# Yotsuei/ClearConverse

Hardware: AMD Instinct MI355X
Metric: xRT (audio-sec/wall-sec) end-to-end, 30 s 16 kHz clips (higher is better)
Workload: dtype bf16

## Files before the change

### clearconverse_amd/csrc/sepformer.hip

```cpp
#include <math.h>
#include "../../include/ccx.h"
#include "ccx_common.h"
#include "elementwise.h"
#include <type_traits>
#include "gemm_bf16.h"
#include "model_store.h"
#include "sepformer.h"

namespace {

typedef __attribute__((ext_vector_type(4))) short bf16x4v;

__global__ __launch_bounds__(256) void sep_encoder_kernel(const float* __restrict__ mix, long mix_stride,
                                                          const int* __restrict__ tok_utt, const int* __restrict__ tok_pos,
                                                          const int* __restrict__ utt_L, const float* __restrict__ w,
                                                          float* __restrict__ feats, int n_tok) {
  const int tok = blockIdx.x * 4 + (threadIdx.x >> 6), lane = threadIdx.x & 63;
  if (tok >= n_tok) return;
  const int u = tok_utt[tok], l = tok_pos[tok];
  float2 o = make_float2(0.f, 0.f);
  if (l < utt_L[u]) {
    const float* x = mix + (long)u * mix_stride + 8 * l;
    float xs[16];
#pragma unroll
    for (int k = 0; k < 16; k++) xs[k] = x[k];
    float a = 0.f, b = 0.f;
#pragma unroll
    for (int k = 0; k < 16; k++) {
      a = fmaf(w[(2 * lane) * 16 + k], xs[k], a);
      b = fmaf(w[(2 * lane + 1) * 16 + k], xs[k], b);
    }
    o = make_float2(fmaxf(a, 0.f), fmaxf(b, 0.f));
  }
  ((float2*)(feats + (long)tok * 128))[lane] = o;
}

__global__ void sep_block_input_kernel(const float* __restrict__ x, const float* __restrict__ hc, const int* __restrict__ tok_seq,
                                       const int* __restrict__ tok_pos, const float* __restrict__ pe, float* __restrict__ xin,
                                       float* __restrict__ h, int n_tok) {
  const long i = (long)blockIdx.x * blockDim.x + threadIdx.x;
  if (i >= (long)n_tok * 32) return;
  const int tok = (int)(i >> 5), c4 = (int)(i & 31);
  float4 v = ((const float4*)x)[i];
  if (hc) {
    const float4 a = ((const float4*)(hc + (long)tok_seq[tok] * 128))[c4];
    v.x += a.x; v.y += a.y; v.z += a.z; v.w += a.w;
  }
  ((float4*)xin)[i] = v;
  const float4 p = ((const float4*)(pe + (long)tok_pos[tok] * 128))[c4];
  ((float4*)h)[i] = make_float4(v.x + p.x, v.y + p.y, v.z + p.z, v.w + p.w);
}

__global__ __launch_bounds__(256, 2) void sep_attention_kernel(const bf16_t* __restrict__ qkv, const int* __restrict__ seq_start,
                                                            const int* __restrict__ seq_len, bf16_t* __restrict__ out,
                                                            float scale_log2e) {
  const int lane = threadIdx.x & 63, wave = threadIdx.x >> 6;
  const int seq = blockIdx.x, head = blockIdx.y * 4 + wave;
  const int s0 = seq_start[seq], len = seq_len[seq];
  const int l15 = lane & 15, h4 = lane >> 4;
  const int n_qt = (len + 15) >> 4, n_kt = n_qt;
  const bf16_t* base = qkv + (long)s0 * 384 + head * 16;

  auto load_k = [&](int kt) -> bf16x4v {
    int krow = kt * 16 + l15;
    krow = krow < len ? krow : len - 1;
    return *(const bf16x4v*)(base + 128 + (long)krow * 384 + 4 * h4);
  };
  auto load_v = [&](int kt) -> bf16x4v {
    bf16x4v v;
#pragma unroll
    for (int j = 0; j < 4; j++) {
      int vr = kt * 16 + 4 * h4 + j;
      vr = vr < len ? vr : len - 1;
      v[j] = (short)base[256 + (long)vr * 384 + l15];
    }
    return v;
  };
  const bool resident = n_kt <= 10;
  bf16x4v k_all[10], v_all[10];
  if (resident) {
#pragma unroll
    for (int t = 0; t < 10; t++) {
      const int kt = t < n_kt ? t : n_kt - 1;
      k_all[t] = load_k(kt);
      v_all[t] = load_v(kt);
    }
  }

  for (int qt = 0; qt < n_qt; qt++) {
    int qrow = qt * 16 + l15;
    qrow = qrow < len ? qrow : len - 1;
    const bf16x4v qf = *(const bf16x4v*)(base + (long)qrow * 384 + 4 * h4);
    float m_run = -1e30f, l_run = 0.f;
    f32x4 o = {0.f, 0.f, 0.f, 0.f};
    auto key_block = [&](int kt0, int nk, auto full_tag) {
      constexpr bool FULL = decltype(full_tag)::value;
      f32x4 s[10];
      bf16x4v vf[10];
#pragma unroll
      for (int t = 0; t < 10; t++) {
        if (FULL || t < nk) {
          const bf16x4v kf = resident ? k_all[t] : load_k(kt0 + t);
          s[t] = __builtin_amdgcn_mfma_f32_16x16x16bf16_1k(kf, qf, (f32x4){0.f, 0.f, 0.f, 0.f}, 0, 0, 0);
          vf[t] = resident ? v_all[t] : load_v(kt0 + t);
        }
      }
      float mx = -1e30f;
#pragma unroll
      for (int t = 0; t < 10; t++)
        if (FULL || t < nk) {
          if ((kt0 + t) * 16 + 16 > len) {
#pragma unroll
            for (int r = 0; r < 4; r++)
              if ((kt0 + t) * 16 + 4 * h4 + r >= len) s[t][r] = -INFINITY;
          }
#pragma unroll
          for (int r = 0; r < 4; r++) mx = fmaxf(mx, s[t][r]);
        }
      mx = fmaxf(mx, lane_xor16(mx));
      mx = fmaxf(mx, lane_xor32(mx));
      mx = fmaxf(m_run, mx * scale_log2e);
      const float alpha = __builtin_amdgcn_exp2f(m_run - mx);
      m_run = mx;
      float ps = 0.f;
#pragma unroll
      for (int t = 0; t < 10; t++)
        if (FULL || t < nk) {
#pragma unroll
          for (int r = 0; r < 4; r++) {
            const float pv = __builtin_amdgcn_exp2f(fmaf(s[t][r], scale_log2e, -mx));
            s[t][r] = pv;
            ps += pv;
          }
        }
      l_run = l_run * alpha + ps;
      float arow[4];
#pragma unroll
      for (int r = 0; r < 4; r++) arow[r] = __shfl(alpha, 4 * h4 + r, 64);
#pragma unroll
      for (int r = 0; r < 4; r++) o[r] *= arow[r];
#pragma unroll
      for (int t = 0; t < 10; t++)
        if (FULL || t < nk) {
          union { bf16x4v v; uint32_t u[2]; } pa;
          pa.u[0] = pack_bf16x2(s[t][0], s[t][1]);
          pa.u[1] = pack_bf16x2(s[t][2], s[t][3]);
          o = __builtin_amdgcn_mfma_f32_16x16x16bf16_1k(pa.v, vf[t], o, 0, 0, 0);
        }
    };
    for (int kt0 = 0; kt0 < n_kt; kt0 += 10) {
      const int nk = (n_kt - kt0) < 10 ? (n_kt - kt0) : 10;
      if (nk == 10) key_block(kt0, 10, std::true_type{});
      else key_block(kt0, nk, std::false_type{});
    }
    float lt = l_run + lane_xor16(l_run);
    lt += lane_xor32(lt);
#pragma unroll
    for (int r = 0; r < 4; r++) {
      const int q = qt * 16 + 4 * h4 + r;
      const float inv = 1.0f / __shfl(lt, 4 * h4 + r, 64);
      if (q < len) out[(long)(s0 + q) * 128 + head * 16 + l15] = f32_to_bf16(o[r] * inv);
    }
  }
}

__device__ __forceinline__ float2 ln_row128(const float* __restrict__ row, const float* __restrict__ g,
                                            const float* __restrict__ b, int lane) {
  const float2 v = ((const float2*)row)[lane];
  const float mean = wave_reduce_sum(v.x + v.y) * (1.0f / 128.0f);
  const float dx = v.x - mean, dy = v.y - mean;
  const float rstd = rsqrtf(wave_reduce_sum(dx * dx + dy * dy) * (1.0f / 128.0f) + 1e-6f);
  const float2 gg = ((const float2*)g)[lane], bb = ((const float2*)b)[lane];
  return make_float2(dx * rstd * gg.x + bb.x, dy * rstd * gg.y + bb.y);
}

__global__ __launch_bounds__(256) void sep_final_norm_kernel(const float* __restrict__ h, const float* __restrict__ xin,
                                                             const int* __restrict__ seq_start, const int* __restrict__ seq_len,
                                                             const float* __restrict__ ln_g, const float* __restrict__ ln_b,
                                                             const float* __restrict__ gln_g, const float* __restrict__ gln_b,
                                                             float* __restrict__ y) {
  __shared__ float red[8];
  const int seq = blockIdx.x, lane = threadIdx.x & 63, wave = threadIdx.x >> 6;
  const int s0 = seq_start[seq], len = seq_len[seq];
  float sum = 0.f;
  for (int r = wave; r < len; r += 4) {
    const float2 v = ln_row128(h + (long)(s0 + r) * 128, ln_g, ln_b, lane);
    sum += v.x + v.y;
  }
  sum = wave_reduce_sum(sum);
  if (lane == 0) red[wave] = sum;
  __syncthreads();
  const float n = (float)len * 128.0f;
  const float mean = (red[0] + red[1] + red[2] + red[3]) / n;
  float sq = 0.f;
  for (int r = wave; r < len; r += 4) {
    const float2 v = ln_row128(h + (long)(s0 + r) * 128, ln_g, ln_b, lane);
    sq += (v.x - mean) * (v.x - mean) + (v.y - mean) * (v.y - mean);
  }
  sq = wave_reduce_sum(sq);
  if (lane == 0) red[4 + wave] = sq;
  __syncthreads();
  const float rstd = 1.0f / sqrtf((red[4] + red[5] + red[6] + red[7]) / n + 1e-8f);
  const float2 gg = ((const float2*)gln_g)[lane], bb = ((const float2*)gln_b)[lane];
  for (int r = wave; r < len; r += 4) {
    const float2 v = ln_row128(h + (long)(s0 + r) * 128, ln_g, ln_b, lane);
    const float2 xi = ((const float2*)(xin + (long)(s0 + r) * 128))[lane];
    ((float2*)(y + (long)(s0 + r) * 128))[lane] =
        make_float2(gg.x * (v.x - mean) * rstd + bb.x + xi.x, gg.y * (v.y - mean) * rstd + bb.y + xi.y);
  }
}

#define FF_TOK 256
#define FF_HB 64
#define FF_P1 (FF_HB * 256)
#define FF_P2 (128 * FF_HB * 2)
#define FF_STAGE (FF_P1 + FF_P2)
#define FF_NSTAGE 4
#define FF_LDS (FF_NSTAGE * FF_STAGE + 4096)
typedef const __attribute__((address_space(1))) void* ff_gptr_t;
typedef __attribute__((address_space(3))) void* ff_lptr_t;

__device__ __forceinline__ int ff_key1(int r) { return (r & 3) | (((r >> 4) & 3) << 2); }
__device__ __forceinline__ int ff_key2(int r) { return ((r >> 1) & 1) | (((r >> 5) & 1) << 2); }

constexpr int AB_MAX_TOK = CCX_SEP_FUSED_MAX_TOK;
__device__ __forceinline__ int ab_off(int row, int chunk) { return row * 256 + ((chunk ^ (row & 15)) << 4); }

__global__ __launch_bounds__(512) void sep_attn_block_kernel(float* __restrict__ h, const float* __restrict__ ln_g, const float* __restrict__ ln_b,
                                                             const bf16_t* __restrict__ Wqkv, const float* __restrict__ bqkv,
                                                             const bf16_t* __restrict__ Wo, const float* __restrict__ bo,
                                                             const int* __restrict__ seq_start, const int* __restrict__ seq_len,
                                                             float scale_log2e, float eps) {
  __shared__ __attribute__((aligned(16))) char xs[AB_MAX_TOK * 256];
  const int tid = threadIdx.x, lane = tid & 63;
  const int wave = __builtin_amdgcn_readfirstlane(tid >> 6);
  const int l15 = lane & 15, h4 = lane >> 4;
  const int seq = blockIdx.x;
  const int s0 = seq_start[seq], len = seq_len[seq];
  if (len <= 0) return;
  const int n_t = (len + 15) >> 4;

  {
    const float2 g = ((const float2*)ln_g)[lane], b = ((const float2*)ln_b)[lane];
#pragma unroll
    for (int half = 0; half < 2; half++) {
      float2 v[10];
#pragma unroll
      for (int i = 0; i < 10; i++) {
        const int r = wave + 8 * (10 * half + i);
        v[i] = r < len ? ((const float2*)(h + (long)(s0 + r) * 128))[lane] : make_float2(0.f, 0.f);
      }
#pragma unroll
      for (int i = 0; i < 10; i++) {
        const int r = wave + 8 * (10 * half + i);
        const float mean = wave_reduce_sum(v[i].x + v[i].y) * (1.f / 128.f);
        const float dx = v[i].x - mean, dy = v[i].y - mean;
        const float rstd = rsqrtf(wave_reduce_sum(dx * dx + dy * dy) * (1.f / 128.f) + eps);
        uint32_t o = pack_bf16x2(dx * rstd * g.x + b.x, dy * rstd * g.y + b.y);
        if (r >= len) o = 0;
        *(uint32_t*)(xs + ab_off(r, lane >> 2) + (lane & 3) * 4) = o;
      }
    }
  }
  __syncthreads();

  bf16x4v q_all[10], k_all[10], v_all[10];
  {
    bf16x8 wq[4], wk[4];
#pragma unroll
    for (int ks = 0; ks < 4; ks++) {
      const long o = (long)(16 * wave + l15) * 128 + 32 * ks + 8 * h4;
      wq[ks] = *(const bf16x8*)(Wqkv + o);
      wk[ks] = *(const bf16x8*)(Wqkv + 128 * 128 + o);
    }
    const float4 bq = *(const float4*)(bqkv + 16 * wave + 4 * h4);
    const float4 bk = *(const float4*)(bqkv + 128 + 16 * wave + 4 * h4);
#pragma unroll
    for (int t = 0; t < 10; t++) {
      const int tt = t < n_t ? t : n_t - 1;
      f32x4 aq = {0.f, 0.f, 0.f, 0.f}, ak = aq;
#pragma unroll
      for (int ks = 0; ks < 4; ks++) {
        const bf16x8 xf = *(const bf16x8*)(xs + ab_off(16 * tt + l15, 4 * ks + h4));
        aq = __builtin_amdgcn_mfma_f32_16x16x32_bf16(wq[ks], xf, aq, 0, 0, 0);
        ak = __builtin_amdgcn_mfma_f32_16x16x32_bf16(wk[ks], xf, ak, 0, 0, 0);
      }
      union { bf16x4v v; uint32_t u[2]; } c;
      c.u[0] = pack_bf16x2(aq[0] + bq.x, aq[1] + bq.y); c.u[1] = pack_bf16x2(aq[2] + bq.z, aq[3] + bq.w);
      q_all[t] = c.v;
      c.u[0] = pack_bf16x2(ak[0] + bk.x, ak[1] + bk.y); c.u[1] = pack_bf16x2(ak[2] + bk.z, ak[3] + bk.w);
      k_all[t] = c.v;
    }
  }
  {
    bf16x8 wv[4];
#pragma unroll
    for (int ks = 0; ks < 4; ks++) wv[ks] = *(const bf16x8*)(Wqkv + 256 * 128 + (long)(16 * wave + l15) * 128 + 32 * ks + 8 * h4);
    const float bv = bqkv[256 + 16 * wave + l15];
#pragma unroll
    for (int t = 0; t < 10; t++) {
      const int tt = t < n_t ? t : n_t - 1;
      f32x4 av = {0.f, 0.f, 0.f, 0.f};
#pragma unroll
      for (int ks = 0; ks < 4; ks++) {
        const bf16x8 xf = *(const bf16x8*)(xs + ab_off(16 * tt + l15, 4 * ks + h4));
        av = __builtin_amdgcn_mfma_f32_16x16x32_bf16(xf, wv[ks], av, 0, 0, 0);
      }
      union { bf16x4v v; uint32_t u[2]; } c;
      c.u[0] = pack_bf16x2(av[0] + bv, av[1] + bv); c.u[1] = pack_bf16x2(av[2] + bv, av[3] + bv);
      v_all[t] = c.v;
    }
  }
  __syncthreads();

  for (int qt = 0; qt < n_t; qt++) {
    bf16x4v qf = q_all[0];
#pragma unroll
    for (int t = 1; t < 10; t++) qf = (t == qt) ? q_all[t] : qf;
    f32x4 sc[10];
#pragma unroll
    for (int t = 0; t < 10; t++) sc[t] = __builtin_amdgcn_mfma_f32_16x16x16bf16_1k(k_all[t], qf, (f32x4){0.f, 0.f, 0.f, 0.f}, 0, 0, 0);
    float mx = -1e30f;
#pragma unroll
    for (int t = 0; t < 10; t++) {
      if (t * 16 + 16 > len) {
#pragma unroll
        for (int r = 0; r < 4; r++)
          if (t * 16 + 4 * h4 + r >= len) sc[t][r] = -INFINITY;
      }
#pragma unroll
      for (int r = 0; r < 4; r++) mx = fmaxf(mx, sc[t][r]);
    }
    mx = fmaxf(mx, lane_xor16(mx));
    mx = fmaxf(mx, lane_xor32(mx));
    mx *= scale_log2e;
    float ps = 0.f;
    f32x4 o = {0.f, 0.f, 0.f, 0.f};
#pragma unroll
    for (int t = 0; t < 10; t++) {
#pragma unroll
      for (int r = 0; r < 4; r++) {
        const float pv = __builtin_amdgcn_exp2f(fmaf(sc[t][r], scale_log2e, -mx));
        sc[t][r] = pv;
        ps += pv;
      }
      union { bf16x4v v; uint32_t u[2]; } pa;
      pa.u[0] = pack_bf16x2(sc[t][0], sc[t][1]);
      pa.u[1] = pack_bf16x2(sc[t][2], sc[t][3]);
      o = __builtin_amdgcn_mfma_f32_16x16x16bf16_1k(pa.v, v_all[t], o, 0, 0, 0);
    }
    float lt = ps + lane_xor16(ps);
    lt += lane_xor32(lt);
#pragma unroll
    for (int r = 0; r < 4; r++) {
      const int row = qt * 16 + 4 * h4 + r;
      const float inv = 1.0f / __shfl(lt, 4 * h4 + r, 64);
      *(bf16_t*)(xs + ab_off(row, 2 * wave + (l15 >> 3)) + (l15 & 7) * 2) = f32_to_bf16(o[r] * inv);
    }
  }
  __syncthreads();

  {
    bf16x8 wo[4];
#pragma unroll
    for (int ks = 0; ks < 4; ks++) wo[ks] = *(const bf16x8*)(Wo + (long)(16 * wave + l15) * 128 + 32 * ks + 8 * h4);
    const float4 b4 = *(const float4*)(bo + 16 * wave + 4 * h4);
    for (int t = 0; t < n_t; t++) {
      const int tok = 16 * t + l15;
      float4* hp = (float4*)(h + (long)(s0 + (tok < len ? tok : len - 1)) * 128 + 16 * wave + 4 * h4);
      const float4 res = *hp;
      f32x4 acc = {0.f, 0.f, 0.f, 0.f};
#pragma unroll
      for (int ks = 0; ks < 4; ks++) {
        const bf16x8 af = *(const bf16x8*)(xs + ab_off(tok, 4 * ks + h4));
        acc = __builtin_amdgcn_mfma_f32_16x16x32_bf16(wo[ks], af, acc, 0, 0, 0);
      }
      if (tok < len) *hp = make_float4(res.x + acc[0] + b4.x, res.y + acc[1] + b4.y, res.z + acc[2] + b4.z, res.w + acc[3] + b4.w);
    }
  }
}

__global__ __launch_bounds__(512) void sep_ffn_kernel(float* __restrict__ h, const float* __restrict__ ln_g, const float* __restrict__ ln_b,
                                                      const bf16_t* __restrict__ W1, const float* __restrict__ b1,
                                                      const bf16_t* __restrict__ W2, const float* __restrict__ b2, int n_tok, int d_ffn,
                                                      float eps) {
  extern __shared__ __attribute__((aligned(16))) char ff_smem[];
  const int tid = threadIdx.x, lane = tid & 63, wave = tid >> 6;
  const int l15 = lane & 15, hq = lane >> 4;
  const int tok0 = blockIdx.x * FF_TOK + wave * 32;
  const int n_stage = d_ffn / FF_HB;
  float* b1s = (float*)(ff_smem + FF_NSTAGE * FF_STAGE);

  const bf16_t* src1[2];
  const bf16_t* src2[2];
#pragma unroll
  for (int i = 0; i < 2; i++) {
    const int r1 = (wave * 2 + i) * 4 + (lane >> 4);
    src1[i] = W1 + (long)r1 * 128 + (((lane & 15) ^ ff_key1(r1)) << 3);
    const int r2 = (wave * 2 + i) * 8 + (lane >> 3);
    src2[i] = W2 + (long)r2 * d_ffn + (((lane & 7) ^ ff_key2(r2)) << 3);
  }
  auto stage = [&](int st) {
    char* s1 = ff_smem + (st & (FF_NSTAGE - 1)) * FF_STAGE;
    char* s2 = s1 + FF_P1;
#pragma unroll
    for (int i = 0; i < 2; i++)
      __builtin_amdgcn_global_load_lds((ff_gptr_t)(src1[i] + (long)st * FF_HB * 128), (ff_lptr_t)(s1 + (wave * 2 + i) * 1024), 16, 0, 0);
#pragma unroll
    for (int i = 0; i < 2; i++)
      __builtin_amdgcn_global_load_lds((ff_gptr_t)(src2[i] + (long)st * FF_HB), (ff_lptr_t)(s2 + (wave * 2 + i) * 1024), 16, 0, 0);
  };

  bf16x8 xb[2][4];
  {
    float g[32], bt[32];
#pragma unroll
    for (int ob = 0; ob < 2; ob++)
#pragma unroll
      for (int i4 = 0; i4 < 4; i4++) {
        const float4 gv = ((const float4*)(ln_g + 64 * ob + 16 * hq))[i4], bv = ((const float4*)(ln_b + 64 * ob + 16 * hq))[i4];
        g[16 * ob + 4 * i4] = gv.x; g[16 * ob + 4 * i4 + 1] = gv.y; g[16 * ob + 4 * i4 + 2] = gv.z; g[16 * ob + 4 * i4 + 3] = gv.w;
        bt[16 * ob + 4 * i4] = bv.x; bt[16 * ob + 4 * i4 + 1] = bv.y; bt[16 * ob + 4 * i4 + 2] = bv.z; bt[16 * ob + 4 * i4 + 3] = bv.w;
      }
#pragma unroll
    for (int mt = 0; mt < 2; mt++) {
      int tok = tok0 + mt * 16 + l15;
      tok = tok < n_tok ? tok : n_tok - 1;
      const float* xr = h + (long)tok * 128 + 16 * hq;
      float v[32];
#pragma unroll
      for (int ob = 0; ob < 2; ob++)
#pragma unroll
        for (int i4 = 0; i4 < 4; i4++) {
          const float4 t = ((const float4*)(xr + 64 * ob))[i4];
          v[16 * ob + 4 * i4] = t.x; v[16 * ob + 4 * i4 + 1] = t.y; v[16 * ob + 4 * i4 + 2] = t.z; v[16 * ob + 4 * i4 + 3] = t.w;
        }
      float sm = 0.f;
#pragma unroll
      for (int c = 0; c < 32; c++) sm += v[c];
      sm += lane_xor16(sm); sm += lane_xor32(sm);
      const float mean = sm * (1.f / 128.f);
      float sq = 0.f;
#pragma unroll
      for (int c = 0; c < 32; c++) { const float d = v[c] - mean; sq = fmaf(d, d, sq); }
      sq += lane_xor16(sq); sq += lane_xor32(sq);
      const float rstd = rsqrtf(sq * (1.f / 128.f) + eps);
#pragma unroll
      for (int ks = 0; ks < 4; ks++) {
        union { bf16x8 vv; uint32_t u[4]; } cv;
#pragma unroll
        for (int e = 0; e < 4; e++) {
          const int c = 8 * ks + 2 * e;
          cv.u[e] = pack_bf16x2((v[c] - mean) * rstd * g[c] + bt[c], (v[c + 1] - mean) * rstd * g[c + 1] + bt[c + 1]);
        }
        xb[mt][ks] = cv.vv;
      }
    }
  }
  for (int i = tid; i < d_ffn; i += 512) b1s[i] = b1[i];

  f32x4 acc2[2][8];
#pragma unroll
  for (int mt = 0; mt < 2; mt++)
#pragma unroll
    for (int jo = 0; jo < 8; jo++) acc2[mt][jo] = (f32x4){0.f, 0.f, 0.f, 0.f};

  const int rq = 16 * (l15 >> 2) + (l15 & 3);
  const int k1 = l15;
  const int k2 = ((l15 >> 1) & 1) | (((l15 >> 3) & 1) << 2);
  asm volatile("s_waitcnt vmcnt(0)" ::: "memory");
  stage(0);
  if (n_stage > 1) stage(1);
  if (n_stage > 2) stage(2);
  for (int st = 0; st < n_stage; st++) {
    const int ahead = n_stage - 1 - st;
    if (ahead >= 2) asm volatile("s_waitcnt vmcnt(8)" ::: "memory");
    else if (ahead == 1) asm volatile("s_waitcnt vmcnt(4)" ::: "memory");
    else asm volatile("s_waitcnt vmcnt(0)" ::: "memory");
    asm volatile("s_waitcnt lgkmcnt(0)" ::: "memory");
    __builtin_amdgcn_s_barrier();
    if (st + 3 < n_stage) stage(st + 3);
    const char* s1 = ff_smem + (st & (FF_NSTAGE - 1)) * FF_STAGE;
    const char* s2 = s1 + FF_P1;
    f32x4 acc1[2][4];
    f32x4 bv[4];
    {
      const uint32_t baddr = (uint32_t)(uintptr_t)(ff_lptr_t)(b1s + st * FF_HB + 16 * hq);
#pragma unroll
      for (int j = 0; j < 4; j++) asm volatile("ds_read_b128 %0, %1" : "=v"(bv[j]) : "v"(baddr + 16 * j) : "memory");
    }
#pragma unroll
    for (int mt = 0; mt < 2; mt++)
#pragma unroll
      for (int j = 0; j < 4; j++) acc1[mt][j] = (f32x4){0.f, 0.f, 0.f, 0.f};
#pragma unroll
    for (int ks = 0; ks < 4; ks++) {
      const int chunk = 8 * (ks >> 1) + 2 * hq + (ks & 1);
#pragma unroll
      for (int j = 0; j < 4; j++) {
        const bf16x8 w = *(const bf16x8*)(s1 + (rq + 4 * j) * 256 + ((chunk ^ k1) << 4));
        acc1[0][j] = __builtin_amdgcn_mfma_f32_16x16x32_bf16(w, xb[0][ks], acc1[0][j], 0, 0, 0);
        acc1[1][j] = __builtin_amdgcn_mfma_f32_16x16x32_bf16(w, xb[1][ks], acc1[1][j], 0, 0, 0);
      }
    }
    asm volatile("s_waitcnt lgkmcnt(0)" ::: "memory");
    __builtin_amdgcn_sched_barrier(0);
    bf16x8 sf[2][2];
#pragma unroll
    for (int mt = 0; mt < 2; mt++)
#pragma unroll
      for (int sx = 0; sx < 2; sx++) {
        union { bf16x8 vv; uint32_t u[4]; } cv;
        const f32x4 a = acc1[mt][2 * sx] + bv[2 * sx], b = acc1[mt][2 * sx + 1] + bv[2 * sx + 1];
        cv.u[0] = pack_bf16x2(fmaxf(a[0], 0.f), fmaxf(a[1], 0.f)); cv.u[1] = pack_bf16x2(fmaxf(a[2], 0.f), fmaxf(a[3], 0.f));
        cv.u[2] = pack_bf16x2(fmaxf(b[0], 0.f), fmaxf(b[1], 0.f)); cv.u[3] = pack_bf16x2(fmaxf(b[2], 0.f), fmaxf(b[3], 0.f));
        sf[mt][sx] = cv.vv;
      }
#pragma unroll
    for (int sx = 0; sx < 2; sx++) {
      const int chunk = 2 * hq + sx;
#pragma unroll
      for (int jo = 0; jo < 8; jo++) {
        const bf16x8 w = *(const bf16x8*)(s2 + (64 * (jo >> 2) + rq + 4 * (jo & 3)) * 128 + ((chunk ^ k2) << 4));
        acc2[0][jo] = __builtin_amdgcn_mfma_f32_16x16x32_bf16(w, sf[0][sx], acc2[0][jo], 0, 0, 0);
        acc2[1][jo] = __builtin_amdgcn_mfma_f32_16x16x32_bf16(w, sf[1][sx], acc2[1][jo], 0, 0, 0);
      }
    }
  }

#pragma unroll
  for (int mt = 0; mt < 2; mt++) {
    const int tok = tok0 + mt * 16 + l15;
    if (tok >= n_tok) continue;
#pragma unroll
    for (int ob = 0; ob < 2; ob++) {
      float4* hp = (float4*)(h + (long)tok * 128 + 64 * ob + 16 * hq);
      const float4* bp = (const float4*)(b2 + 64 * ob + 16 * hq);
#pragma unroll
      for (int jp = 0; jp < 4; jp++) {
        const float4 r = hp[jp], bv = bp[jp];
        const f32x4 a = acc2[mt][4 * ob + jp];
        hp[jp] = make_float4(a[0] + bv.x + r.x, a[1] + bv.y + r.y, a[2] + bv.z + r.z, a[3] + bv.w + r.w);
      }
    }
  }
}

__global__ __launch_bounds__(128) void sep_chunk_mean_kernel(const float* __restrict__ x, float* __restrict__ mem, int seg) {
  const int chunk = blockIdx.x, c = threadIdx.x;
  const float* p = x + (long)chunk * seg * 128 + c;
  float s = 0.f;
  for (int t = 0; t < seg; t++) s += p[(long)t * 128];
  mem[(long)chunk * 128 + c] = s / (float)seg;
}

__global__ void sep_prelu_bf16_kernel(const float* __restrict__ x, const float* __restrict__ slope, bf16_t* __restrict__ out, long n4) {
  const long i = (long)blockIdx.x * blockDim.x + threadIdx.x;
  if (i >= n4) return;
  const float a = slope[0];
  const float4 v = ((const float4*)x)[i];
  uint2 o;
  o.x = pack_bf16x2(v.x >= 0 ? v.x : a * v.x, v.y >= 0 ? v.y : a * v.y);
  o.y = pack_bf16x2(v.z >= 0 ? v.z : a * v.z, v.w >= 0 ? v.w : a * v.w);
  ((uint2*)out)[i] = o;
}

__global__ __launch_bounds__(256) void sep_decoder_kernel(const float* __restrict__ feats, const float* __restrict__ fc,
                                                          const int* __restrict__ utt_tok0, const int* __restrict__ utt_L,
                                                          const int* __restrict__ utt_T, const float* __restrict__ wdec,
                                                          float* __restrict__ out, long out_stride, int n_utt) {
  const int u = blockIdx.y;
  const int l = blockIdx.x * 4 + (threadIdx.x >> 6), lane = threadIdx.x & 63;
  const int T = utt_T[u], L = utt_L[u];
  const long t0 = 8L * l;
  if (t0 >= out_stride) return;
  float2* dst = (float2*)(out + ((long)u * out_stride + t0) * 2);
  if (t0 >= T || l > L) {
    if (lane < 8 && t0 + lane < out_stride) dst[lane] = make_float2(0.f, 0.f);
    return;
  }
  float g[2][2][2];
#pragma unroll
  for (int dl = 0; dl < 2; dl++) {
    const int ll = l - dl;
    const bool ok = ll >= 0 && ll < L;
    const long tok = utt_tok0[u] + (ok ? ll : 0);
    const float2 f = ((const float2*)(feats + tok * 128))[lane];
    const float4 m = ((const float4*)(fc + tok * 256))[lane];
    const float z = ok ? 1.f : 0.f;
    g[dl][0][0] = z * f.x * fmaxf(m.x, 0.f); g[dl][0][1] = z * f.y * fmaxf(m.z, 0.f);
    g[dl][1][0] = z * f.x * fmaxf(m.y, 0.f); g[dl][1][1] = z * f.y * fmaxf(m.w, 0.f);
  }
  float4 w0[4], w1[4];
#pragma unroll
  for (int i = 0; i < 4; i++) {
    w0[i] = ((const float4*)(wdec + (2 * lane) * 16))[i];
    w1[i] = ((const float4*)(wdec + (2 * lane + 1) * 16))[i];
  }
  const float* w0f = (const float*)w0;
  const float* w1f = (const float*)w1;
  float2 res = make_float2(0.f, 0.f);
#pragma unroll
  for (int k = 0; k < 8; k++) {
    float a0 = g[0][0][0] * w0f[k] + g[0][0][1] * w1f[k];
    float a1 = g[0][1][0] * w0f[k] + g[0][1][1] * w1f[k];
    a0 += g[1][0][0] * w0f[k + 8] + g[1][0][1] * w1f[k + 8];
    a1 += g[1][1][0] * w0f[k + 8] + g[1][1][1] * w1f[k + 8];
    a0 = wave_reduce_sum(a0);
    a1 = wave_reduce_sum(a1);
    if (lane == k) res = make_float2(a0, a1);
  }
  if (lane < 8 && t0 + lane < out_stride) dst[lane] = (t0 + lane < T) ? res : make_float2(0.f, 0.f);
}

struct SepLayer {
  float *ln1_g, *ln1_b, *ln2_g, *ln2_b, *bqkv, *bo, *b1, *b2;
  bf16_t *Wqkv, *Wo, *W1, *W2;
};
struct SepBlock {
  std::vector<SepLayer> layers;
  float *lnf_g, *lnf_b, *gln_g, *gln_b;
};

}

static constexpr float kSepScaleLog2e = 0.25f * 1.4426950408889634f;
static constexpr float kSepLnEps = 1e-6f;

int ccx_launch_sep_attn_block(ccx_ctx* ctx, float* h, const float* ln_g, const float* ln_b, const bf16_t* Wqkv, const float* bqkv,
                              const bf16_t* Wo, const float* bo, const int* seq_start, const int* seq_len, int n_seq, int n_tok,
                              int max_len, hipStream_t st) {
  const int D = 128;
  {
    ccx_prof_scope ps(ctx, st, "sep_attn_block_kernel", 2.0 * n_tok * (double)D * 4 * D + 4.0 * n_tok * (double)max_len * D,
                      2.0 * n_tok * D * 4.0 + 2.0 * 4 * D * D);
    hipLaunchKernelGGL(sep_attn_block_kernel, dim3(n_seq), dim3(512), 0, st, h, ln_g, ln_b, Wqkv, bqkv, Wo, bo, seq_start, seq_len,
                       kSepScaleLog2e, kSepLnEps);
  }
  CCX_CHECK_LAUNCH(ctx);
  return CCX_OK;
}

int ccx_launch_sep_attention(ccx_ctx* ctx, const bf16_t* qkv, const int* seq_start, const int* seq_len, int n_seq, int n_head,
                             bf16_t* out, hipStream_t st) {
  {
    ccx_prof_scope ps(ctx, st, "sep_attention_kernel", 0.0, 0.0);
    hipLaunchKernelGGL(sep_attention_kernel, dim3(n_seq, n_head / 4), dim3(256), 0, st, qkv, seq_start, seq_len, out, kSepScaleLog2e);
  }
  CCX_CHECK_LAUNCH(ctx);
  return CCX_OK;
}

int ccx_launch_sep_ffn(ccx_ctx* ctx, float* h, const float* ln_g, const float* ln_b, const bf16_t* W1, const float* b1,
                       const bf16_t* W2, const float* b2, int n_tok, int d_ffn, hipStream_t st) {
  const int D = 128;
  {
    static ccx_lds_optin optin;
    CCX_HIP(ctx, optin.ensure(ctx->device, (const void*)sep_ffn_kernel, FF_LDS));
    ccx_prof_scope ps(ctx, st, "sep_ffn_kernel", 4.0 * n_tok * (double)D * d_ffn, 2.0 * n_tok * D * 4.0 + 4.0 * D * d_ffn);
    hipLaunchKernelGGL(sep_ffn_kernel, dim3(ccx_cdiv(n_tok, FF_TOK)), dim3(512), FF_LDS, st, h, ln_g, ln_b, W1, b1, W2, b2, n_tok, d_ffn,
                       kSepLnEps);
  }
  CCX_CHECK_LAUNCH(ctx);
  return CCX_OK;
}

int ccx_launch_sep_final_norm(ccx_ctx* ctx, const float* h, const float* xin, const int* seq_start, const int* seq_len, int n_seq,
                              const float* ln_g, const float* ln_b, const float* gln_g, const float* gln_b, float* y, hipStream_t st) {
  hipLaunchKernelGGL(sep_final_norm_kernel, dim3(n_seq), dim3(256), 0, st, h, xin, seq_start, seq_len, ln_g, ln_b, gln_g, gln_b, y);
  CCX_CHECK_LAUNCH(ctx);
  return CCX_OK;
}

int ccx_launch_sep_decoder(ccx_ctx* ctx, const float* feats, const float* fc, const int* utt_tok0, const int* utt_L, const int* utt_T,
                           const float* wdec, float* out, long out_stride, int n_utt, hipStream_t st) {
  hipLaunchKernelGGL(sep_decoder_kernel, dim3(ccx_cdiv(ccx_cdiv((int)out_stride, 8), 4), n_utt), dim3(256), 0, st, feats, fc, utt_tok0, utt_L,
                     utt_T, wdec, out, out_stride, n_utt);
  CCX_CHECK_LAUNCH(ctx);
  return CCX_OK;
}

struct ccx_sepformer {
  ccx_ctx* ctx = nullptr;
  ccx_sepformer_dims d{};
  int max_tokens = 0, max_utts = 0;
  bool finalized = false;
  ccx_dev_store store{"sepformer"};
  float *w_enc = nullptr, *w_dec = nullptr, *prelu = nullptr, *b_fc = nullptr, *pe = nullptr;
  bf16_t* W_fc = nullptr;
  std::vector<SepBlock> seg, mem;
  float *feats = nullptr, *x = nullptr, *xin = nullptr, *h = nullptr, *fc = nullptr, *memx = nullptr, *memxin = nullptr,
        *memh = nullptr, *hc = nullptr;
  bf16_t *xn = nullptr, *qkv = nullptr, *att = nullptr;
  int *tok_utt = nullptr, *tok_pos = nullptr, *tok_chunk = nullptr, *tok_cpos = nullptr, *chunk_start = nullptr,
      *chunk_len = nullptr, *utt_L = nullptr, *utt_T = nullptr, *utt_tok0 = nullptr, *utt_chunk0 = nullptr, *utt_nchunk = nullptr,
      *mem_utt = nullptr, *mem_pos = nullptr;
  int pe_len = 0;
};

namespace {

int load_block(ccx_sepformer* s, const std::string& prefix, SepBlock& B) {
  const int D = s->d.d_model, F = s->d.d_ffn;
  B.layers.resize(s->d.n_layers);
  for (int l = 0; l < s->d.n_layers; l++) {
    const std::string p = prefix + ".mdl.layers." + std::to_string(l);
    SepLayer& L = B.layers[l];
    CCX_NEED(s->store, wi, p + ".self_att.att.in_proj_weight", 3 * D, D); CCX_NEED(s->store, bi, p + ".self_att.att.in_proj_bias", 3 * D);
    CCX_NEED(s->store, wo, p + ".self_att.att.out_proj.weight", D, D); CCX_NEED(s->store, bo, p + ".self_att.att.out_proj.bias", D);
    CCX_NEED(s->store, w1, p + ".pos_ffn.ffn.0.weight", F, D); CCX_NEED(s->store, b1, p + ".pos_ffn.ffn.0.bias", F);
    CCX_NEED(s->store, w2, p + ".pos_ffn.ffn.3.weight", D, F); CCX_NEED(s->store, b2, p + ".pos_ffn.ffn.3.bias", D);
    CCX_NEED(s->store, g1, p + ".norm1.norm.weight", D); CCX_NEED(s->store, be1, p + ".norm1.norm.bias", D);
    CCX_NEED(s->store, g2, p + ".norm2.norm.weight", D); CCX_NEED(s->store, be2, p + ".norm2.norm.bias", D);
    CCX_TRY(s->store.upload_bf16(&L.Wqkv, wi->data)); CCX_TRY(s->store.upload(&L.bqkv, bi->data.data(), 3 * D));
    CCX_TRY(s->store.upload_bf16(&L.Wo, wo->data)); CCX_TRY(s->store.upload(&L.bo, bo->data.data(), D));
    CCX_TRY(s->store.upload_bf16(&L.W1, w1->data)); CCX_TRY(s->store.upload(&L.b1, b1->data.data(), F));
    CCX_TRY(s->store.upload_bf16(&L.W2, w2->data)); CCX_TRY(s->store.upload(&L.b2, b2->data.data(), D));
    CCX_TRY(s->store.upload(&L.ln1_g, g1->data.data(), D)); CCX_TRY(s->store.upload(&L.ln1_b, be1->data.data(), D));
    CCX_TRY(s->store.upload(&L.ln2_g, g2->data.data(), D)); CCX_TRY(s->store.upload(&L.ln2_b, be2->data.data(), D));
  }
  CCX_NEED(s->store, fg, prefix + ".mdl.norm.norm.weight", D); CCX_NEED(s->store, fb, prefix + ".mdl.norm.norm.bias", D);
  CCX_NEED(s->store, gg, prefix + ".norm.weight", D); CCX_NEED(s->store, gb, prefix + ".norm.bias", D);
  CCX_TRY(s->store.upload(&B.lnf_g, fg->data.data(), D)); CCX_TRY(s->store.upload(&B.lnf_b, fb->data.data(), D));
  CCX_TRY(s->store.upload(&B.gln_g, gg->data.data(), D)); CCX_TRY(s->store.upload(&B.gln_b, gb->data.data(), D));
  return CCX_OK;
}

int run_block(ccx_sepformer* s, const SepBlock& B, const float* x, const float* hc, const int* tok_seq, const int* tok_pos,
              const int* seq_start, const int* seq_len, int n_tok, int n_seq, int max_len, float* xin, float* h, float* y, hipStream_t st) {
  ccx_ctx* ctx = s->ctx;
  const int D = s->d.d_model, F = s->d.d_ffn;
  hipLaunchKernelGGL(sep_block_input_kernel, dim3(ccx_cdiv(n_tok * 32, 256)), dim3(256), 0, st, x, hc, tok_seq, tok_pos, s->pe,
                     xin, h, n_tok);
  CCX_CHECK_LAUNCH(ctx);
  const char* fenv = getenv("CCX_SEP_FUSED_ATTN");
  const bool fused = (fenv ? atoi(fenv) != 0 : true) && max_len <= AB_MAX_TOK;
  for (const SepLayer& L : B.layers) {
    GemmParams p;
    if (fused) {
      CCX_TRY(ccx_launch_sep_attn_block(ctx, h, L.ln1_g, L.ln1_b, L.Wqkv, L.bqkv, L.Wo, L.bo, seq_start, seq_len, n_seq, n_tok, max_len, st));
    } else {
    CCX_TRY(ccx_launch_layernorm(ctx, h, D, L.ln1_g, L.ln1_b, s->xn, nullptr, D, n_tok, D, 1e-6f, st));
    memset(&p, 0, sizeof(p));
    p.A = s->xn; p.lda = D; p.W = L.Wqkv; p.ldw = D; p.M = n_tok; p.N = 3 * D; p.K = D; p.bias = L.bqkv; p.out = s->qkv; p.ldo = 3 * D;
    CCX_TRY(ccx_launch_gemm(ctx, EPI_BF16, p, st));
    CCX_TRY(ccx_launch_sep_attention(ctx, s->qkv, seq_start, seq_len, n_seq, s->d.n_head, s->att, st));
    memset(&p, 0, sizeof(p));
    p.A = s->att; p.lda = D; p.W = L.Wo; p.ldw = D; p.M = n_tok; p.N = D; p.K = D; p.bias = L.bo; p.out = h; p.ldo = D; p.resid = h; p.ldr = D;
    CCX_TRY(ccx_launch_gemm(ctx, EPI_F32_RESID, p, st));
    }
    CCX_TRY(ccx_launch_sep_ffn(ctx, h, L.ln2_g, L.ln2_b, L.W1, L.b1, L.W2, L.b2, n_tok, F, st));
  }
  CCX_TRY(ccx_launch_sep_final_norm(ctx, h, xin, seq_start, seq_len, n_seq, B.lnf_g, B.lnf_b, B.gln_g, B.gln_b, y, st));
  return CCX_OK;
}

}

extern "C" {

int ccx_sepformer_create(ccx_ctx* ctx, const ccx_sepformer_dims* dims, int max_tokens, int max_utts, ccx_sepformer** out) {
  if (!ctx) return CCX_ERR_ARG;
  CCX_REQUIRE(ctx, dims && out, "ccx_sepformer_create: null argument");
  const ccx_sepformer_dims& d = *dims;
  CCX_REQUIRE(ctx, d.n_filters == 128 && d.d_model == 128 && d.kernel == 16 && d.stride == 8 && d.n_head == 8 && d.n_spk == 2,
              "sepformer: only the resepformer-wsj02mix geometry (128 filters, k16 s8, d_model 128, 8 heads, 2 speakers) is built");
  CCX_REQUIRE(ctx, d.d_ffn % 128 == 0 && d.d_ffn <= 1024 && d.segment >= 16 && d.n_layers >= 1 && d.n_blocks >= 1, "sepformer: bad dims");
  CCX_REQUIRE(ctx, max_tokens >= d.segment && max_utts >= 1, "sepformer: capacity too small");
  ccx_sepformer* s = new ccx_sepformer();
  s->ctx = ctx; s->store.ctx = ctx; s->d = d;
  s->max_tokens = ccx_cdiv(max_tokens, d.segment) * d.segment;
  s->max_utts = max_utts;
  *out = s;
  return CCX_OK;
}

void ccx_sepformer_destroy(ccx_sepformer* s) {
  if (!s) return;
  s->store.free_all();
  delete s;
}

int ccx_sepformer_set_tensor(ccx_sepformer* s, const char* name, const float* data, int64_t numel) {
  if (!s) return CCX_ERR_ARG;
  CCX_REQUIRE(s->ctx, !s->finalized && name && data && numel > 0, "sepformer: set_tensor bad arguments");
  const std::string nm(name);
  CCX_REQUIRE(s->ctx, nm.rfind("encoder.", 0) == 0 || nm.rfind("decoder.", 0) == 0 || nm.rfind("masknet.", 0) == 0,
              "sepformer: unknown tensor name '%s'", name);
  return s->store.stage(name, data, numel);
}

int ccx_sepformer_finalize(ccx_sepformer* s) {
  if (!s) return CCX_ERR_ARG;
  CCX_REQUIRE(s->ctx, !s->finalized, "sepformer: finalize called twice");
  const ccx_sepformer_dims& d = s->d;
  const int D = d.d_model, F = d.d_ffn, N = d.n_filters;
  {
    CCX_NEED(s->store, we, "encoder.conv1d.weight", N, 1, d.kernel);
    CCX_NEED(s->store, wd, "decoder.weight", N, 1, d.kernel);
    CCX_NEED(s->store, pr, "masknet.model.output_fc.0.weight", 1);
    CCX_NEED(s->store, wf, "masknet.model.output_fc.1.weight", N * d.n_spk, D, 1);
    CCX_NEED(s->store, bf, "masknet.model.output_fc.1.bias", N * d.n_spk);
    CCX_TRY(s->store.upload(&s->w_enc, we->data));
    CCX_TRY(s->store.upload(&s->w_dec, wd->data));
    CCX_TRY(s->store.upload(&s->prelu, pr->data.data(), 1));
    CCX_TRY(s->store.upload_bf16(&s->W_fc, wf->data));
    CCX_TRY(s->store.upload(&s->b_fc, bf->data));
  }
  s->seg.resize(d.n_blocks);
  s->mem.resize(d.n_blocks > 0 ? d.n_blocks - 1 : 0);
  for (int i = 0; i < d.n_blocks; i++) {
    CCX_TRY(load_block(s, "masknet.model.seg_model." + std::to_string(i), s->seg[i]));
    if (i < d.n_blocks - 1) CCX_TRY(load_block(s, "masknet.model.mem_model." + std::to_string(i), s->mem[i]));
  }
  s->store.staged.clear();
  const int max_chunks = s->max_tokens / d.segment;
  s->pe_len = d.segment > max_chunks ? d.segment : max_chunks;
  {
    std::vector<float> pe((size_t)s->pe_len * D);
    for (int p = 0; p < s->pe_len; p++)
      for (int i = 0; i < D; i += 2) {
        const float den = expf((float)i * -(logf(10000.0f) / (float)D));
        pe[(size_t)p * D + i] = sinf((float)p * den);
        pe[(size_t)p * D + i + 1] = cosf((float)p * den);
      }
    CCX_TRY(s->store.upload(&s->pe, pe));
  }
  const size_t T = (size_t)s->max_tokens;
  CCX_TRY(s->store.alloc(&s->feats, T * D, true)); CCX_TRY(s->store.alloc(&s->x, T * D, true)); CCX_TRY(s->store.alloc(&s->xin, T * D, true)); CCX_TRY(s->store.alloc(&s->h, T * D, true));
  CCX_TRY(s->store.alloc(&s->fc, T * 2 * D, true)); CCX_TRY(s->store.alloc(&s->xn, T * D, true)); CCX_TRY(s->store.alloc(&s->qkv, T * 3 * D, true));
  CCX_TRY(s->store.alloc(&s->att, T * D, true));
  CCX_TRY(s->store.alloc(&s->memx, (size_t)max_chunks * D, true)); CCX_TRY(s->store.alloc(&s->memxin, (size_t)max_chunks * D, true));
  CCX_TRY(s->store.alloc(&s->memh, (size_t)max_chunks * D, true)); CCX_TRY(s->store.alloc(&s->hc, (size_t)max_chunks * D, true));
  CCX_TRY(s->store.alloc(&s->tok_utt, T, true)); CCX_TRY(s->store.alloc(&s->tok_pos, T, true)); CCX_TRY(s->store.alloc(&s->tok_chunk, T, true)); CCX_TRY(s->store.alloc(&s->tok_cpos, T, true));
  CCX_TRY(s->store.alloc(&s->chunk_start, (size_t)max_chunks, true)); CCX_TRY(s->store.alloc(&s->chunk_len, (size_t)max_chunks, true));
  CCX_TRY(s->store.alloc(&s->mem_utt, (size_t)max_chunks, true)); CCX_TRY(s->store.alloc(&s->mem_pos, (size_t)max_chunks, true));
  const size_t U = (size_t)s->max_utts;
  CCX_TRY(s->store.alloc(&s->utt_L, U, true)); CCX_TRY(s->store.alloc(&s->utt_T, U, true)); CCX_TRY(s->store.alloc(&s->utt_tok0, U, true)); CCX_TRY(s->store.alloc(&s->utt_chunk0, U, true));
  CCX_TRY(s->store.alloc(&s->utt_nchunk, U, true));
  s->finalized = true;
  return CCX_OK;
}

int ccx_sepformer_separate(ccx_sepformer* s, const float* mix, int64_t stride, const int* n_samples, int B, float* out,
                           void* stream_) {
  if (!s) return CCX_ERR_ARG;
  ccx_ctx* ctx = s->ctx;
  hipStream_t st = (hipStream_t)stream_;
  CCX_REQUIRE(ctx, s->finalized && mix && n_samples && out && B >= 1 && B <= s->max_utts, "sepformer_separate: bad arguments (B=%d, max %d)", B, s->max_utts);
  const ccx_sepformer_dims& d = s->d;
  const int D = d.d_model, seg = d.segment;
  std::vector<int> uL(B), uT(B), utok0(B), uchunk0(B), unchunk(B);
  int n_tok = 0, n_chunk = 0, max_nchunk = 0;
  for (int b = 0; b < B; b++) {
    CCX_REQUIRE(ctx, n_samples[b] >= d.kernel && n_samples[b] <= stride, "sepformer_separate: utterance %d has %d samples (need >= %d, <= stride)", b, n_samples[b], d.kernel);
    uT[b] = n_samples[b];
    uL[b] = (n_samples[b] - d.kernel) / d.stride + 1;
    const int rest = seg - uL[b] % seg;
    unchunk[b] = (uL[b] + rest) / seg;
    utok0[b] = n_tok; uchunk0[b] = n_chunk;
    n_tok += unchunk[b] * seg; n_chunk += unchunk[b];
    max_nchunk = unchunk[b] > max_nchunk ? unchunk[b] : max_nchunk;
  }
  CCX_REQUIRE(ctx, n_tok <= s->max_tokens, "sepformer_separate: %d tokens exceed capacity %d", n_tok, s->max_tokens);
  CCX_REQUIRE(ctx, n_chunk <= s->pe_len, "sepformer_separate: memory sequence too long");
  std::vector<int> t_utt(n_tok), t_pos(n_tok), t_chunk(n_tok), t_cpos(n_tok), c_start(n_chunk), c_len(n_chunk), m_utt(n_chunk), m_pos(n_chunk);
  for (int b = 0; b < B; b++) {
    for (int c = 0; c < unchunk[b]; c++) {
      const int cg = uchunk0[b] + c;
      c_start[cg] = utok0[b] + c * seg; c_len[cg] = seg; m_utt[cg] = b; m_pos[cg] = c;
      for (int i = 0; i < seg; i++) {
        const int t = c_start[cg] + i;
        t_utt[t] = b; t_pos[t] = c * seg + i; t_chunk[t] = cg; t_cpos[t] = i;
      }
    }
  }
#define UP(dst, vec) CCX_HIP(ctx, hipMemcpyAsync(dst, vec.data(), vec.size() * 4, hipMemcpyHostToDevice, st))
  UP(s->tok_utt, t_utt); UP(s->tok_pos, t_pos); UP(s->tok_chunk, t_chunk); UP(s->tok_cpos, t_cpos);
  UP(s->chunk_start, c_start); UP(s->chunk_len, c_len); UP(s->mem_utt, m_utt); UP(s->mem_pos, m_pos);
  UP(s->utt_L, uL); UP(s->utt_T, uT); UP(s->utt_tok0, utok0); UP(s->utt_chunk0, uchunk0); UP(s->utt_nchunk, unchunk);
#undef UP
  CCX_HIP(ctx, hipStreamSynchronize(st));

  hipLaunchKernelGGL(sep_encoder_kernel, dim3(ccx_cdiv(n_tok, 4)), dim3(256), 0, st, mix, (long)stride, s->tok_utt, s->tok_pos,
                     s->utt_L, s->w_enc, s->feats, n_tok);
  CCX_CHECK_LAUNCH(ctx);
  const float* cur = s->feats;
  const float* hc = nullptr;
  for (int i = 0; i < d.n_blocks; i++) {
    CCX_TRY(run_block(s, s->seg[i], cur, hc, s->tok_chunk, s->tok_cpos, s->chunk_start, s->chunk_len, n_tok, n_chunk, seg, s->xin, s->h,
                   s->x, st));
    cur = s->x;
    if (i < d.n_blocks - 1) {
      hipLaunchKernelGGL(sep_chunk_mean_kernel, dim3(n_chunk), dim3(128), 0, st, s->x, s->memx, seg);
      CCX_CHECK_LAUNCH(ctx);
      CCX_TRY(run_block(s, s->mem[i], s->memx, nullptr, s->mem_utt, s->mem_pos, s->utt_chunk0, s->utt_nchunk, n_chunk, B, max_nchunk, s->memxin,
                     s->memh, s->hc, st));
      hc = s->hc;
    }
  }
  hipLaunchKernelGGL(sep_prelu_bf16_kernel, dim3(ccx_cdiv(n_tok * 32, 256)), dim3(256), 0, st, s->x, s->prelu, s->xn, (long)n_tok * 32);
  CCX_CHECK_LAUNCH(ctx);
  GemmParams p;
  memset(&p, 0, sizeof(p));
  p.A = s->xn; p.lda = D; p.W = s->W_fc; p.ldw = D; p.M = n_tok; p.N = 2 * D; p.K = D; p.bias = s->b_fc; p.out = s->fc; p.ldo = 2 * D;
  CCX_TRY(ccx_launch_gemm(ctx, EPI_F32, p, st));
  return ccx_launch_sep_decoder(ctx, s->feats, s->fc, s->utt_tok0, s->utt_L, s->utt_T, s->w_dec, out, (long)stride, B, st);
}

}
```

Measured before the change: 1698.

## Restructure attention block kernel to prefetch weights and residuals early

Loads the K/V weights and biases before LayerNorm and fuses the K and V projections into one loop over tiles. Q weights load partway through that loop, and Q tiles go to shared memory instead of being selected from registers. The Wo weights and residual rows are prefetched before the barrier, and the output projection is fully unrolled with stores deferred. The aim is to hide global-load latency and cut register-select overhead, with a launch bound of 4 and asm pins to steer register allocation. The cost is higher register pressure and full 10-tile unrolling even for short sequences.

```diff
diff --git a/clearconverse_amd/csrc/sepformer.hip b/clearconverse_amd/csrc/sepformer.hip
--- a/clearconverse_amd/csrc/sepformer.hip
+++ b/clearconverse_amd/csrc/sepformer.hip
@@ -226,7 +226,9 @@
 constexpr int AB_MAX_TOK = CCX_SEP_FUSED_MAX_TOK;
 __device__ __forceinline__ int ab_off(int row, int chunk) { return row * 256 + ((chunk ^ (row & 15)) << 4); }
 
-__global__ __launch_bounds__(512) void sep_attn_block_kernel(float* __restrict__ h, const float* __restrict__ ln_g, const float* __restrict__ ln_b,
+#define AB_PIN(a, b) asm volatile("" : "+v"(a), "+v"(b))
+
+__global__ __launch_bounds__(512, 4) void sep_attn_block_kernel(float* __restrict__ h, const float* __restrict__ ln_g, const float* __restrict__ ln_b,
                                                              const bf16_t* __restrict__ Wqkv, const float* __restrict__ bqkv,
                                                              const bf16_t* __restrict__ Wo, const float* __restrict__ bo,
                                                              const int* __restrict__ seq_start, const int* __restrict__ seq_len,
@@ -240,6 +242,16 @@
   if (len <= 0) return;
   const int n_t = (len + 15) >> 4;
 
+  bf16x8 wk[4], wv[4];
+#pragma unroll
+  for (int ks = 0; ks < 4; ks++) {
+    const long o = (long)(16 * wave + l15) * 128 + 32 * ks + 8 * h4;
+    wk[ks] = *(const bf16x8*)(Wqkv + 128 * 128 + o);
+    wv[ks] = *(const bf16x8*)(Wqkv + 256 * 128 + o);
+  }
+  const float4 bk = *(const float4*)(bqkv + 128 + 16 * wave + 4 * h4);
+  const float bv = bqkv[256 + 16 * wave + l15];
+
   {
     const float2 g = ((const float2*)ln_g)[lane], b = ((const float2*)ln_b)[lane];
 #pragma unroll
@@ -262,61 +274,55 @@
       }
     }
   }
+  const float4 bq = *(const float4*)(bqkv + 16 * wave + 4 * h4);
   __syncthreads();
 
   bf16x4v q_all[10], k_all[10], v_all[10];
-  {
-    bf16x8 wq[4], wk[4];
+  bf16x8 wq[4];
+#pragma unroll
+  for (int t = 0; t < 10; t++) {
+    if (t == 7) {
+#pragma unroll
+      for (int ks = 0; ks < 4; ks++) wq[ks] = *(const bf16x8*)(Wqkv + (long)(16 * wave + l15) * 128 + 32 * ks + 8 * h4);
+    }
+    f32x4 ak = {0.f, 0.f, 0.f, 0.f}, av = ak;
 #pragma unroll
     for (int ks = 0; ks < 4; ks++) {
-      const long o = (long)(16 * wave + l15) * 128 + 32 * ks + 8 * h4;
-      wq[ks] = *(const bf16x8*)(Wqkv + o);
-      wk[ks] = *(const bf16x8*)(Wqkv + 128 * 128 + o);
-    }
-    const float4 bq = *(const float4*)(bqkv + 16 * wave + 4 * h4);
-    const float4 bk = *(const float4*)(bqkv + 128 + 16 * wave + 4 * h4);
-#pragma unroll
-    for (int t = 0; t < 10; t++) {
-      const int tt = t < n_t ? t : n_t - 1;
-      f32x4 aq = {0.f, 0.f, 0.f, 0.f}, ak = aq;
-#pragma unroll
-      for (int ks = 0; ks < 4; ks++) {
-        const bf16x8 xf = *(const bf16x8*)(xs + ab_off(16 * tt + l15, 4 * ks + h4));
-        aq = __builtin_amdgcn_mfma_f32_16x16x32_bf16(wq[ks], xf, aq, 0, 0, 0);
-        ak = __builtin_amdgcn_mfma_f32_16x16x32_bf16(wk[ks], xf, ak, 0, 0, 0);
-      }
-      union { bf16x4v v; uint32_t u[2]; } c;
-      c.u[0] = pack_bf16x2(aq[0] + bq.x, aq[1] + bq.y); c.u[1] = pack_bf16x2(aq[2] + bq.z, aq[3] + bq.w);
-      q_all[t] = c.v;
-      c.u[0] = pack_bf16x2(ak[0] + bk.x, ak[1] + bk.y); c.u[1] = pack_bf16x2(ak[2] + bk.z, ak[3] + bk.w);
-      k_all[t] = c.v;
-    }
-  }
-  {
-    bf16x8 wv[4];
-#pragma unroll
-    for (int ks = 0; ks < 4; ks++) wv[ks] = *(const bf16x8*)(Wqkv + 256 * 128 + (long)(16 * wave + l15) * 128 + 32 * ks + 8 * h4);
-    const float bv = bqkv[256 + 16 * wave + l15];
-#pragma unroll
-    for (int t = 0; t < 10; t++) {
-      const int tt = t < n_t ? t : n_t - 1;
-      f32x4 av = {0.f, 0.f, 0.f, 0.f};
-#pragma unroll
-      for (int ks = 0; ks < 4; ks++) {
-        const bf16x8 xf = *(const bf16x8*)(xs + ab_off(16 * tt + l15, 4 * ks + h4));
-        av = __builtin_amdgcn_mfma_f32_16x16x32_bf16(xf, wv[ks], av, 0, 0, 0);
-      }
-      union { bf16x4v v; uint32_t u[2]; } c;
-      c.u[0] = pack_bf16x2(av[0] + bv, av[1] + bv); c.u[1] = pack_bf16x2(av[2] + bv, av[3] + bv);
-      v_all[t] = c.v;
-    }
-  }
+      const bf16x8 xf = *(const bf16x8*)(xs + ab_off(16 * t + l15, 4 * ks + h4));
+      ak = __builtin_amdgcn_mfma_f32_16x16x32_bf16(wk[ks], xf, ak, 0, 0, 0);
+      av = __builtin_amdgcn_mfma_f32_16x16x32_bf16(xf, wv[ks], av, 0, 0, 0);
+    }
+    union { bf16x4v v; uint32_t u[2]; } c;
+    c.u[0] = pack_bf16x2(ak[0] + bk.x, ak[1] + bk.y); c.u[1] = pack_bf16x2(ak[2] + bk.z, ak[3] + bk.w);
+    AB_PIN(c.u[0], c.u[1]);
+    k_all[t] = c.v;
+    c.u[0] = pack_bf16x2(av[0] + bv, av[1] + bv); c.u[1] = pack_bf16x2(av[2] + bv, av[3] + bv);
+    AB_PIN(c.u[0], c.u[1]);
+    v_all[t] = c.v;
+  }
+#pragma unroll
+  for (int t = 0; t < 10; t++) {
+    f32x4 aq = {0.f, 0.f, 0.f, 0.f};
+#pragma unroll
+    for (int ks = 0; ks < 4; ks++) {
+      const bf16x8 xf = *(const bf16x8*)(xs + ab_off(16 * t + l15, 4 * ks + h4));
+      aq = __builtin_amdgcn_mfma_f32_16x16x32_bf16(wq[ks], xf, aq, 0, 0, 0);
+    }
+    union { bf16x4v v; uint32_t u[2]; } c;
+    c.u[0] = pack_bf16x2(aq[0] + bq.x, aq[1] + bq.y); c.u[1] = pack_bf16x2(aq[2] + bq.z, aq[3] + bq.w);
+    AB_PIN(c.u[0], c.u[1]);
+    q_all[t] = c.v;
+  }
+  bf16x8 wo[4];
+#pragma unroll
+  for (int ks = 0; ks < 4; ks++) wo[ks] = *(const bf16x8*)(Wo + (long)(16 * wave + l15) * 128 + 32 * ks + 8 * h4);
   __syncthreads();
 
+#pragma unroll
+  for (int t = 0; t < 10; t++) *(bf16x4v*)(xs + ab_off(16 * t + l15, 2 * wave + (h4 >> 1)) + (h4 & 1) * 8) = q_all[t];
+
   for (int qt = 0; qt < n_t; qt++) {
-    bf16x4v qf = q_all[0];
-#pragma unroll
-    for (int t = 1; t < 10; t++) qf = (t == qt) ? q_all[t] : qf;
+    const bf16x4v qf = *(const bf16x4v*)(xs + ab_off(16 * qt + l15, 2 * wave + (h4 >> 1)) + (h4 & 1) * 8);
     f32x4 sc[10];
 #pragma unroll
     for (int t = 0; t < 10; t++) sc[t] = __builtin_amdgcn_mfma_f32_16x16x16bf16_1k(k_all[t], qf, (f32x4){0.f, 0.f, 0.f, 0.f}, 0, 0, 0);
@@ -358,25 +364,33 @@
       *(bf16_t*)(xs + ab_off(row, 2 * wave + (l15 >> 3)) + (l15 & 7) * 2) = f32_to_bf16(o[r] * inv);
     }
   }
+  float4 b4 = *(const float4*)(bo + 16 * wave + 4 * h4);
+  float4 res[10];
+#pragma unroll
+  for (int t = 0; t < 10; t++) {
+    const int tok = 16 * t + l15;
+    res[t] = *(const float4*)(h + (long)(s0 + (tok < len ? tok : len - 1)) * 128 + 16 * wave + 4 * h4);
+  }
   __syncthreads();
 
-  {
-    bf16x8 wo[4];
-#pragma unroll
-    for (int ks = 0; ks < 4; ks++) wo[ks] = *(const bf16x8*)(Wo + (long)(16 * wave + l15) * 128 + 32 * ks + 8 * h4);
-    const float4 b4 = *(const float4*)(bo + 16 * wave + 4 * h4);
-    for (int t = 0; t < n_t; t++) {
-      const int tok = 16 * t + l15;
-      float4* hp = (float4*)(h + (long)(s0 + (tok < len ? tok : len - 1)) * 128 + 16 * wave + 4 * h4);
-      const float4 res = *hp;
-      f32x4 acc = {0.f, 0.f, 0.f, 0.f};
-#pragma unroll
-      for (int ks = 0; ks < 4; ks++) {
-        const bf16x8 af = *(const bf16x8*)(xs + ab_off(tok, 4 * ks + h4));
-        acc = __builtin_amdgcn_mfma_f32_16x16x32_bf16(wo[ks], af, acc, 0, 0, 0);
-      }
-      if (tok < len) *hp = make_float4(res.x + acc[0] + b4.x, res.y + acc[1] + b4.y, res.z + acc[2] + b4.z, res.w + acc[3] + b4.w);
-    }
+  asm volatile("" : "+v"(b4.x), "+v"(b4.y), "+v"(b4.z), "+v"(b4.w));
+  int l15o = l15;
+  asm volatile("" : "+v"(l15o));
+#pragma unroll
+  for (int t = 0; t < 10; t++) {
+    const int tok = 16 * t + l15o;
+    f32x4 acc = {0.f, 0.f, 0.f, 0.f};
+#pragma unroll
+    for (int ks = 0; ks < 4; ks++) {
+      const bf16x8 af = *(const bf16x8*)(xs + ab_off(tok, 4 * ks + h4));
+      acc = __builtin_amdgcn_mfma_f32_16x16x32_bf16(wo[ks], af, acc, 0, 0, 0);
+    }
+    res[t] = make_float4(res[t].x + acc[0] + b4.x, res[t].y + acc[1] + b4.y, res[t].z + acc[2] + b4.z, res[t].w + acc[3] + b4.w);
+  }
+#pragma unroll
+  for (int t = 0; t < 10; t++) {
+    const int tok = 16 * t + l15o;
+    if (tok < len) *(float4*)(h + (long)(s0 + tok) * 128 + 16 * wave + 4 * h4) = res[t];
   }
 }
 
```

Result: no change. 1709, median of 6 (+0.7%).
